# Consensys/gnark

Measured on AMD Instinct MI355X. Metric: G1 MSM throughput, BN254, 2^24 scalar-muls on one GPU (Groth16 proofs/s at 2^24 constraints in 'groth16'), higher is better.
Workload: dtype u64 Montgomery limbs in memory; 29/28-bit limbs, v_mad_u64_u32 (32x32+64) in registers

## Files before the change

### gnark_amd/csrc/msm_reduce.hip.h

```cpp
#pragma once
#include <vector>

#include "msm_lazy.hip.h"

namespace ga {

constexpr int MSM_HOT_TASKS = 16;
constexpr uint32_t MSM_VHOT_TASKS = 512;
constexpr uint32_t MSM_VHOT_SPLIT = 64;
constexpr int MSM_GROUP = 32;

template <class F>
__global__ void __launch_bounds__(64)
msm_hot_kernel(const XYZZ<F>* __restrict__ partial, const uint32_t* __restrict__ task_off,
               const uint32_t* __restrict__ hot_list, const uint32_t* __restrict__ hot_count, XYZZ<F>* __restrict__ bsum,
               uint32_t bsum_stride, uint32_t part_stride) {
    __shared__ LazyPt<F> sh[64];
    __shared__ XYZZ<F> shx[64];
    __shared__ uint32_t bad;
    partial += (uint64_t)blockIdx.y * part_stride;
    bsum += (uint64_t)blockIdx.y * bsum_stride;
    const uint32_t nh = *hot_count;
    for (uint32_t h = blockIdx.x; h < nh; h += gridDim.x) {
        const uint32_t b = hot_list[h];
        const uint32_t t0 = task_off[b], t1 = task_off[b + 1];
        block_sum29<F>(t1 - t0, [&](uint32_t i) { return &partial[t0 + i]; }, &bsum[b], sh, shx, &bad);
    }
}

template <class F>
__global__ void __launch_bounds__(64)
msm_vhot_stage1_kernel(const XYZZ<F>* __restrict__ partial, const uint32_t* __restrict__ task_off, const uint32_t* __restrict__ vhot_list,
                       const uint32_t* __restrict__ vhot_count, XYZZ<F>* __restrict__ vtmp, uint32_t part_stride, uint32_t vtmp_stride) {
    __shared__ LazyPt<F> sh[64];
    __shared__ XYZZ<F> shx[64];
    __shared__ uint32_t bad;
    partial += (uint64_t)blockIdx.y * part_stride;
    vtmp += (uint64_t)blockIdx.y * vtmp_stride;
    const uint32_t items = *vhot_count * MSM_VHOT_SPLIT;
    for (uint32_t id = blockIdx.x; id < items; id += gridDim.x) {
        const uint32_t h = id / MSM_VHOT_SPLIT, part = id % MSM_VHOT_SPLIT;
        const uint32_t b = vhot_list[h];
        const uint32_t t0 = task_off[b], t1 = task_off[b + 1];
        const uint32_t per = (t1 - t0 + MSM_VHOT_SPLIT - 1) / MSM_VHOT_SPLIT;
        const uint32_t lo = t0 + part * per < t1 ? t0 + part * per : t1;
        const uint32_t hi = lo + per < t1 ? lo + per : t1;
        block_sum29<F>(hi - lo, [&](uint32_t i) { return &partial[lo + i]; }, &vtmp[id], sh, shx, &bad);
    }
}
template <class F>
__global__ void __launch_bounds__(64)
msm_vhot_stage2_kernel(const XYZZ<F>* __restrict__ vtmp, const uint32_t* __restrict__ vhot_list, const uint32_t* __restrict__ vhot_count,
                       XYZZ<F>* __restrict__ bsum, uint32_t bsum_stride, uint32_t vtmp_stride) {
    static_assert(MSM_VHOT_SPLIT == 64, "one partial result per lane");
    __shared__ LazyPt<F> sh[64];
    __shared__ XYZZ<F> shx[64];
    __shared__ uint32_t bad;
    vtmp += (uint64_t)blockIdx.y * vtmp_stride;
    bsum += (uint64_t)blockIdx.y * bsum_stride;
    const uint32_t nv = *vhot_count;
    for (uint32_t h = blockIdx.x; h < nv; h += gridDim.x)
        block_sum29<F>(MSM_VHOT_SPLIT, [&](uint32_t i) { return &vtmp[h * MSM_VHOT_SPLIT + i]; }, &bsum[vhot_list[h]], sh, shx, &bad);
}

template <class F>
__global__ void msm_merge_kernel(const XYZZ<F>* __restrict__ partial, const uint32_t* __restrict__ task_off, uint32_t nb,
                                 XYZZ<F>* __restrict__ bsum, uint32_t* __restrict__ hot_list, uint32_t* __restrict__ hot_count,
                                 uint32_t* __restrict__ vhot_list, uint32_t* __restrict__ vhot_count, uint32_t part_stride) {
    uint32_t b = blockIdx.x * blockDim.x + threadIdx.x;
    if (b >= nb) return;
    partial += (uint64_t)blockIdx.y * part_stride;
    bsum += (uint64_t)blockIdx.y * nb;
    uint32_t t0 = task_off[b], t1 = task_off[b + 1];
    uint32_t nt = t1 - t0;
    if (nt == 1) return;
    if (nt > MSM_VHOT_TASKS) {
        if (blockIdx.y == 0) vhot_list[atomicAdd(vhot_count, 1u)] = b;
        return;
    }
    if (nt > MSM_HOT_TASKS) {
        if (blockIdx.y == 0) hot_list[atomicAdd(hot_count, 1u)] = b;
        return;
    }
    XYZZ<F> out = xyzz_inf<F>();
    bool exact = true;
    if constexpr (BaseFieldOf<F>::P::N <= 8) {
        LazyPt<F> acc;
        acc.inf = 1;
        for (uint32_t t = t0; t < t1; t++) lazy_acc<F>(acc, load_pod<XYZZ<F>>(&partial[t]));
        exact = false;
        if (!acc.inf) {
            out.zz = Lazy<F>::to_mem(acc.v.zz);
            exact = is_zero(out.zz);
            out.x = Lazy<F>::to_mem(acc.v.x);
            out.y = Lazy<F>::to_mem(acc.v.y);
            out.zzz = Lazy<F>::to_mem(acc.v.zzz);
        }
    }
    if (exact) {
        out = xyzz_inf<F>();
        for (uint32_t t = t0; t < t1; t++) out = add(out, load_pod<XYZZ<F>>(&partial[t]));
    }
    store_pod(&bsum[b], out);
}

template <class F>
__global__ void __launch_bounds__(64)
msm_reduce_groups_kernel(const XYZZ<F>* __restrict__ bsum, uint32_t half, uint32_t m, uint32_t groups_per_win,
                         uint32_t total_groups, XYZZ<F>* __restrict__ gsum) {
    uint32_t gid = blockIdx.x * blockDim.x + threadIdx.x;
    if (gid >= total_groups) return;
    uint32_t w = gid / groups_per_win, g = gid % groups_per_win;
    const XYZZ<F>* B = bsum + (uint64_t)w * half + (uint64_t)g * m;
    XYZZ<F> running = xyzz_inf<F>(), local = xyzz_inf<F>();
    for (int j = (int)m - 1; j >= 0; j--) {
        running = add(running, load_pod<XYZZ<F>>(&B[j]));
        local = add(local, running);
    }
    uint32_t base = g * m;
    if (base != 0) {
        XYZZ<F> r = xyzz_inf<F>();
        int top = 31 - __clz(base);
        for (int bit = top; bit >= 0; bit--) {
            r = dbl(r);
            if ((base >> bit) & 1) r = add(r, running);
        }
        local = add(local, r);
    }
    store_pod(&gsum[gid], local);
}

template <class F>
__global__ void __launch_bounds__(64)
msm_reduce_groups29_kernel(const XYZZ<F>* __restrict__ bsum, uint32_t half, uint32_t m, uint32_t groups_per_win,
                           uint32_t total_groups, XYZZ<F>* __restrict__ lsum, XYZZ<F>* __restrict__ rsum,
                           uint32_t* __restrict__ redo_list, uint32_t* __restrict__ redo_count) {
    uint32_t gid = blockIdx.x * blockDim.x + threadIdx.x;
    if (gid >= total_groups) return;
    uint32_t w = gid / groups_per_win, g = gid % groups_per_win;
    const XYZZ<F>* B = bsum + (uint64_t)w * half + (uint64_t)g * m;
    Lazy4<F> running, local;
    bool r_inf = true, l_inf = true;
    for (int j = (int)m - 1; j >= 0; j--) {
        XYZZ<F> b = load_pod<XYZZ<F>>(&B[j]);
        if (!is_inf(b)) {
            Lazy4<F> lb = lazy4_from_mem<F>(b);
            if (r_inf) {
                running = lb;
                r_inf = false;
            } else {
                add29<F>(running, lb);
            }
        }
        if (!r_inf) {
            if (l_inf) {
                local = running;
                l_inf = false;
            } else {
                add29<F>(local, running);
            }
        }
    }
    XYZZ<F> lo = xyzz_inf<F>(), ro = xyzz_inf<F>();
    bool bad = false;
    if (!r_inf) {
        ro.zz = Lazy<F>::to_mem(running.zz);
        lo.zz = Lazy<F>::to_mem(local.zz);
        bad = is_zero(ro.zz) | is_zero(lo.zz);
        ro.x = Lazy<F>::to_mem(running.x);
        ro.y = Lazy<F>::to_mem(running.y);
        ro.zzz = Lazy<F>::to_mem(running.zzz);
        lo.x = Lazy<F>::to_mem(local.x);
        lo.y = Lazy<F>::to_mem(local.y);
        lo.zzz = Lazy<F>::to_mem(local.zzz);
    }
    if (bad) {
        redo_list[atomicAdd(redo_count, 1u)] = gid;
        return;
    }
    store_pod(&lsum[gid], lo);
    store_pod(&rsum[gid], ro);
}

template <class F>
__global__ void __launch_bounds__(64)
msm_reduce_groups_redo_kernel(const XYZZ<F>* __restrict__ bsum, uint32_t half, uint32_t m, uint32_t groups_per_win,
                              const uint32_t* __restrict__ redo_list, const uint32_t* __restrict__ redo_count,
                              XYZZ<F>* __restrict__ lsum, XYZZ<F>* __restrict__ rsum) {
    const uint32_t nredo = *redo_count;
    for (uint32_t r = blockIdx.x * blockDim.x + threadIdx.x; r < nredo; r += gridDim.x * blockDim.x) {
        const uint32_t gid = redo_list[r];
        uint32_t w = gid / groups_per_win, g = gid % groups_per_win;
        const XYZZ<F>* B = bsum + (uint64_t)w * half + (uint64_t)g * m;
        XYZZ<F> running = xyzz_inf<F>(), local = xyzz_inf<F>();
        for (int j = (int)m - 1; j >= 0; j--) {
            running = add(running, load_pod<XYZZ<F>>(&B[j]));
            local = add(local, running);
        }
        store_pod(&lsum[gid], local);
        store_pod(&rsum[gid], running);
    }
}

template <class F>
__global__ void __launch_bounds__(64)
msm_bit_partial_kernel(const XYZZ<F>* __restrict__ rsum, const XYZZ<F>* __restrict__ lsum, uint32_t groups_per_win,
                       uint32_t chunk_len, int log_chunk, XYZZ<F>* __restrict__ part) {
    __shared__ LazyPt<F> sh[64];
    __shared__ XYZZ<F> shx[64];
    __shared__ uint32_t bad;
    const uint32_t ch = blockIdx.x, b = blockIdx.y, w = blockIdx.z;
    const uint32_t nbits = gridDim.y, chunks = gridDim.x;
    const uint32_t base = ch * chunk_len;
    const XYZZ<F>* R = rsum + (uint64_t)w * groups_per_win;
    XYZZ<F>* dst = &part[((uint64_t)w * nbits + b) * chunks + ch];
    if (b == nbits - 1) {
        const XYZZ<F>* Lp = lsum + (uint64_t)w * groups_per_win;
        block_sum29<F>(chunk_len, [&](uint32_t i) { return &Lp[base + i]; }, dst, sh, shx, &bad);
    } else if ((int)b >= log_chunk) {
        block_sum29<F>(((base >> b) & 1) ? chunk_len : 0u, [&](uint32_t i) { return &R[base + i]; }, dst, sh, shx, &bad);
    } else {
        block_sum29<F>(chunk_len / 2, [&](uint32_t i) { return &R[base + (((i >> b) << (b + 1)) | (1u << b) | (i & ((1u << b) - 1)))]; }, dst, sh,
                       shx, &bad);
    }
}

template <class F>
__global__ void __launch_bounds__(64)
msm_segment_sum29_kernel(const XYZZ<F>* __restrict__ in, uint32_t seg_len, XYZZ<F>* __restrict__ out) {
    __shared__ LazyPt<F> sh[64];
    __shared__ XYZZ<F> shx[64];
    __shared__ uint32_t bad;
    const uint64_t base = (uint64_t)blockIdx.x * seg_len;
    block_sum29<F>(seg_len, [&](uint32_t i) { return &in[base + i]; }, &out[blockIdx.x], sh, shx, &bad);
}

template <class F>
__global__ void __launch_bounds__(64)
msm_segment_sum_kernel(const XYZZ<F>* __restrict__ in, uint32_t seg_len, XYZZ<F>* __restrict__ out) {
    __shared__ XYZZ<F> sh[64];
    const uint64_t base = (uint64_t)blockIdx.x * seg_len;
    XYZZ<F> acc = xyzz_inf<F>();
    for (uint32_t g = threadIdx.x; g < seg_len; g += 64) acc = add(acc, load_pod<XYZZ<F>>(&in[base + g]));
    acc = wave_tree_sum(acc, sh);
    if (threadIdx.x == 0) store_pod(&out[blockIdx.x], acc);
}

struct MsmReducePlan {
    int nsets;
    uint32_t m_groups;
    uint32_t groups_per_win, total_groups;
    bool big_set, lazy;
};
inline MsmReducePlan msm_reduce_plan(Ctx* ctx, const void* d_bases, const MsmPrepared& P, int ntab) {
    MsmReducePlan R;
    const uint32_t half = P.half;
    R.nsets = ntab > 1 ? ntab : P.nsets;
    const int tuned_group = ctx->tun.msm_group.load(std::memory_order_relaxed);
    R.m_groups = tuned_group ? (uint32_t)tuned_group : (uint32_t)MSM_GROUP;
    const uint64_t min_lanes = 32768;
    while (R.m_groups > 2 && (uint64_t)half * R.nsets / R.m_groups < min_lanes) R.m_groups >>= 1;
    if (R.m_groups > half) R.m_groups = half;
    R.groups_per_win = half / R.m_groups;
    R.total_groups = R.groups_per_win * R.nsets;
    R.big_set = (uint64_t)half * R.nsets >= ctx->tun.reduce_lazy_min;
    const bool dense_set = P.m >= 16ull * (uint64_t)half * (uint64_t)P.nsets && !(P.table && ctx->is_sparse_set(d_bases));
    R.lazy = R.big_set || dense_set;
    return R;
}

template <class F>
struct MsmMerge {
    uint32_t *hot_list, *hot_count, *vhot_list;
    XYZZ<F>* vtmp;
    uint32_t vtmp_stride;
};
template <class F>
int msm_merge_scratch(Ctx* ctx, const MsmPrepared& P, int ntab, hipStream_t st, MsmMerge<F>* M) {
    const uint64_t vhot_cap = P.max_tasks / MSM_VHOT_TASKS + 2;
    GA_CHECK(ctx->scratch_get("msm_hot", ((uint64_t)P.nb + 2) * 4, (void**)&M->hot_list));
    GA_CHECK(ctx->scratch_get("msm_hot_count", 256, (void**)&M->hot_count));
    GA_CHECK(ctx->scratch_get("msm_vhot", vhot_cap * 4, (void**)&M->vhot_list));
    GA_CHECK(ctx->scratch_get("msm_vhot_tmp", (uint64_t)ntab * vhot_cap * MSM_VHOT_SPLIT * sizeof(XYZZ<F>), (void**)&M->vtmp));
    M->vtmp_stride = (uint32_t)(vhot_cap * MSM_VHOT_SPLIT);
    GA_HIP_CHECK(hipMemsetAsync(M->hot_count, 0, 8, st));
    return GA_OK;
}
template <class F>
int msm_merge(Ctx* ctx, const MsmPrepared& P, int ntab, hipStream_t st, const MsmMerge<F>& M, XYZZ<F>* sums) {
    StageTimer tm(ctx, "msm_merge");
    const uint32_t nb = P.nb, part_stride = (uint32_t)P.max_tasks;
    const unsigned ny = (unsigned)ntab;
    XYZZ<F>* bsum = sums;
    const XYZZ<F>* partial = sums + (uint64_t)ntab * nb;
    const uint32_t *task_off = P.task_off, *hot_count = M.hot_count, *vhot_count = M.hot_count + 1;
    hipLaunchKernelGGL((msm_merge_kernel<F>), dim3((nb + 255) / 256, ny), dim3(256), 0, st, partial, task_off, nb, bsum, M.hot_list, M.hot_count,
                       M.vhot_list, M.hot_count + 1, part_stride);
    hipLaunchKernelGGL((msm_hot_kernel<F>), dim3(512, ny), dim3(64), 0, st, partial, task_off, (const uint32_t*)M.hot_list, hot_count, bsum, nb,
                       part_stride);
    hipLaunchKernelGGL((msm_vhot_stage1_kernel<F>), dim3(2048, ny), dim3(64), 0, st, partial, task_off, (const uint32_t*)M.vhot_list, vhot_count,
                       M.vtmp, part_stride, M.vtmp_stride);
    hipLaunchKernelGGL((msm_vhot_stage2_kernel<F>), dim3(256, ny), dim3(64), 0, st, (const XYZZ<F>*)M.vtmp, (const uint32_t*)M.vhot_list,
                       vhot_count, bsum, nb, M.vtmp_stride);
    GA_KERNEL_CHECK();
    return GA_OK;
}

template <class F>
struct MsmRows {
    const XYZZ<F>* d = nullptr;
    int per_set = 1;
    const uint32_t* flagged_groups = nullptr;
};

template <class F>
int msm_reduce_exact(Ctx* ctx, const MsmReducePlan& R, uint32_t half, const XYZZ<F>* bsum, hipStream_t st, MsmRows<F>* rows) {
    XYZZ<F>*gsum, *gsum2, *wsum;
    GA_CHECK(ctx->scratch_get("msm_gsum", (uint64_t)R.total_groups * sizeof(XYZZ<F>), (void**)&gsum));
    GA_CHECK(ctx->scratch_get("msm_gsum2", ((uint64_t)R.total_groups / 1024 + 64) * sizeof(XYZZ<F>), (void**)&gsum2));
    GA_CHECK(ctx->scratch_get("msm_wsum", (uint64_t)R.nsets * sizeof(XYZZ<F>), (void**)&wsum));
    StageTimer tm(ctx, "msm_reduce");
    hipLaunchKernelGGL((msm_reduce_groups_kernel<F>), dim3((R.total_groups + 63) / 64), dim3(64), 0, st, bsum, half, R.m_groups, R.groups_per_win,
                       R.total_groups, gsum);
    const uint32_t sg = 1024;
    if (R.groups_per_win > 2 * sg) {
        const uint32_t nseg = R.groups_per_win / sg;
        hipLaunchKernelGGL((msm_segment_sum_kernel<F>), dim3(nseg * R.nsets), dim3(64), 0, st, (const XYZZ<F>*)gsum, sg, gsum2);
        hipLaunchKernelGGL((msm_segment_sum_kernel<F>), dim3(R.nsets), dim3(64), 0, st, (const XYZZ<F>*)gsum2, nseg, wsum);
    } else {
        hipLaunchKernelGGL((msm_segment_sum_kernel<F>), dim3(R.nsets), dim3(64), 0, st, (const XYZZ<F>*)gsum, R.groups_per_win, wsum);
    }
    GA_KERNEL_CHECK();
    rows->d = wsum;
    return GA_OK;
}

template <class F>
int msm_reduce_lazy(Ctx* ctx, const MsmReducePlan& R, uint32_t half, const XYZZ<F>* bsum, hipStream_t st, MsmRows<F>* rows) {
    const int nbits = ilog2_u64(R.groups_per_win), nsets = R.nsets;
    uint32_t sg = 1024;
    while (sg > 64 && (uint64_t)(R.groups_per_win / sg) * (uint64_t)(nbits + 1) * (uint64_t)nsets < 2048) sg >>= 1;
    const uint32_t chunk_len = R.groups_per_win > sg ? sg : R.groups_per_win;
    const uint32_t chunks = R.groups_per_win / chunk_len;
    const int log_chunk = ilog2_u64(chunk_len);
    XYZZ<F>*gsum, *rsum, *bpart, *bits;
    uint32_t *rg_list, *rg_count;
    GA_CHECK(ctx->scratch_get("msm_gsum", (uint64_t)R.total_groups * sizeof(XYZZ<F>), (void**)&gsum));
    GA_CHECK(ctx->scratch_get("msm_rsum", (uint64_t)R.total_groups * sizeof(XYZZ<F>), (void**)&rsum));
    GA_CHECK(ctx->scratch_get("msm_bpart", ((uint64_t)nsets * (nbits + 1) * chunks + 64) * sizeof(XYZZ<F>), (void**)&bpart));
    GA_CHECK(ctx->scratch_get("msm_bits", ((uint64_t)nsets * (nbits + 1) + 64) * sizeof(XYZZ<F>), (void**)&bits));
    GA_CHECK(ctx->scratch_get("msm_redo_groups", ((uint64_t)R.total_groups + 2) * 4, (void**)&rg_list));
    GA_CHECK(ctx->scratch_get("msm_redo_groups_count", 256, (void**)&rg_count));
    GA_HIP_CHECK(hipMemsetAsync(rg_count, 0, 4, st));
    StageTimer tm(ctx, "msm_reduce");
    hipLaunchKernelGGL((msm_reduce_groups29_kernel<F>), dim3((R.total_groups + 63) / 64), dim3(64), 0, st, bsum, half, R.m_groups,
                       R.groups_per_win, R.total_groups, gsum, rsum, rg_list, rg_count);
    hipLaunchKernelGGL((msm_reduce_groups_redo_kernel<F>), dim3(256), dim3(64), 0, st, bsum, half, R.m_groups, R.groups_per_win,
                       (const uint32_t*)rg_list, (const uint32_t*)rg_count, gsum, rsum);
    hipLaunchKernelGGL((msm_bit_partial_kernel<F>), dim3(chunks, (unsigned)nbits + 1, (unsigned)nsets), dim3(64), 0, st,
                       (const XYZZ<F>*)rsum, (const XYZZ<F>*)gsum, R.groups_per_win, chunk_len, log_chunk, bpart);
    hipLaunchKernelGGL((msm_segment_sum29_kernel<F>), dim3((unsigned)(nsets * (nbits + 1))), dim3(64), 0, st, (const XYZZ<F>*)bpart,
                       chunks, bits);
    GA_KERNEL_CHECK();
    rows->d = bits;
    rows->per_set = nbits + 1;
    rows->flagged_groups = rg_count;
    return GA_OK;
}

template <class F>
XYZZ<F> msm_combine_horner(const XYZZ<F>* ws, int nsets, int c) {
    XYZZ<F> acc = xyzz_inf<F>();
    for (int w = nsets - 1; w >= 0; w--) {
        for (int k = 0; k < c; k++) acc = dbl(acc);
        acc = add(acc, ws[w]);
    }
    return acc;
}
template <class F>
XYZZ<F> msm_combine_set(const XYZZ<F>* hb, int nbits, int log_m) {
    XYZZ<F> acc = xyzz_inf<F>();
    for (int b = nbits - 1; b >= 0; b--) acc = add(dbl(acc), hb[b]);
    for (int k = 0; k < log_m; k++) acc = dbl(acc);
    return add(hb[nbits], acc);
}
template <class F>
XYZZ<F> msm_combine_descent(const XYZZ<F>* hb, int nsets, int nbits, int log_m, int c) {
    const int rows = nbits + 1, top = c * (nsets - 1) + log_m + nbits - 1;
    std::vector<std::vector<const XYZZ<F>*>> at((size_t)top + 1);
    for (int w = 0; w < nsets; w++) {
        at[(size_t)(c * w)].push_back(&hb[(size_t)w * rows + nbits]);
        for (int b = 0; b < nbits; b++) at[(size_t)(c * w + log_m + b)].push_back(&hb[(size_t)w * rows + b]);
    }
    XYZZ<F> acc = xyzz_inf<F>();
    for (int pos = top; pos >= 0; pos--) {
        if (pos != top) acc = dbl(acc);
        for (const XYZZ<F>* t : at[(size_t)pos]) acc = add(acc, *t);
    }
    return acc;
}
template <class F>
void msm_combine(const MsmReducePlan& R, const XYZZ<F>* h, int per_set, int horner_c, XYZZ<F>* out) {
    const int nbits = per_set - 1, log_m = ilog2_u64(R.m_groups);
    if (!R.lazy) {
        if (horner_c > 0) out[0] = msm_combine_horner(h, R.nsets, horner_c);
        else
            for (int w = 0; w < R.nsets; w++) out[w] = h[w];
    } else if (horner_c > 0) {
        out[0] = msm_combine_descent(h, R.nsets, nbits, log_m, horner_c);
    } else {
        for (int w = 0; w < R.nsets; w++) out[w] = msm_combine_set(h + (size_t)w * per_set, nbits, log_m);
    }
}

}
```

Before: 912.9.

## Compact warm buckets before merging and dedupe high-bit partial sums

The merge step is split into a classify kernel and a merge kernel. The classify kernel builds a warm-bucket list using wave-ballot compaction. The merge kernel then walks only that list, so lanes no longer diverge across buckets with 1, hot, or very-hot task counts, and lazy failures are sent to the hot path instead of an exact serial re-add. The bit-partial stage no longer runs one full row per high bit, most of them empty. It computes a single full-chunk row and lets the final kernel choose chunks by bit, which cuts the partial grid from nbits+1 rows to log_chunk+2. Both changes add extra launches and atomics, and the hot list is now sized per table.

Result: no change. 918.6 (median of 6 runs) (+0.6%).

```diff
diff --git a/gnark_amd/csrc/msm_reduce.hip.h b/gnark_amd/csrc/msm_reduce.hip.h
--- a/gnark_amd/csrc/msm_reduce.hip.h
+++ b/gnark_amd/csrc/msm_reduce.hip.h
@@ -64,44 +64,53 @@
 }
 
 template <class F>
-__global__ void msm_merge_kernel(const XYZZ<F>* __restrict__ partial, const uint32_t* __restrict__ task_off, uint32_t nb,
-                                 XYZZ<F>* __restrict__ bsum, uint32_t* __restrict__ hot_list, uint32_t* __restrict__ hot_count,
-                                 uint32_t* __restrict__ vhot_list, uint32_t* __restrict__ vhot_count, uint32_t part_stride) {
-    uint32_t b = blockIdx.x * blockDim.x + threadIdx.x;
-    if (b >= nb) return;
+__global__ void __launch_bounds__(256)
+msm_merge_classify_kernel(const uint32_t* __restrict__ task_off, uint32_t nb, XYZZ<F>* __restrict__ bsum, uint32_t* __restrict__ warm_list,
+                          uint32_t* __restrict__ warm_count, uint32_t* __restrict__ hot_list, uint32_t* __restrict__ hot_count,
+                          uint32_t* __restrict__ vhot_list, uint32_t* __restrict__ vhot_count) {
+    const uint32_t b = blockIdx.x * blockDim.x + threadIdx.x;
+    const uint32_t nt = b < nb ? task_off[b + 1] - task_off[b] : 1;
+    if (nt == 0) store_pod(&bsum[(uint64_t)blockIdx.y * nb + b], xyzz_inf<F>());
+    if (blockIdx.y != 0) return;
+    if (nt > MSM_VHOT_TASKS) vhot_list[atomicAdd(vhot_count, 1u)] = b;
+    else if (nt > (uint32_t)MSM_HOT_TASKS) hot_list[atomicAdd(hot_count, 1u)] = b;
+    const bool warm = nt >= 2 && nt <= (uint32_t)MSM_HOT_TASKS;
+    const unsigned long long mask = __ballot(warm);
+    if (mask == 0) return;
+    const int lane = threadIdx.x & 63, leader = __ffsll(mask) - 1;
+    uint32_t base = 0;
+    if (lane == leader) base = atomicAdd(warm_count, (uint32_t)__popcll(mask));
+    base = __shfl(base, leader);
+    if (warm) warm_list[base + (uint32_t)__popcll(mask & ((1ull << lane) - 1))] = b;
+}
+
+template <class F>
+__global__ void __launch_bounds__(64)
+msm_merge_warm_kernel(const XYZZ<F>* __restrict__ partial, const uint32_t* __restrict__ task_off, const uint32_t* __restrict__ warm_list,
+                      const uint32_t* __restrict__ warm_count, XYZZ<F>* __restrict__ bsum, uint32_t bsum_stride, uint32_t part_stride,
+                      uint32_t* __restrict__ hot_list, uint32_t* __restrict__ hot_count) {
     partial += (uint64_t)blockIdx.y * part_stride;
-    bsum += (uint64_t)blockIdx.y * nb;
-    uint32_t t0 = task_off[b], t1 = task_off[b + 1];
-    uint32_t nt = t1 - t0;
-    if (nt == 1) return;
-    if (nt > MSM_VHOT_TASKS) {
-        if (blockIdx.y == 0) vhot_list[atomicAdd(vhot_count, 1u)] = b;
-        return;
-    }
-    if (nt > MSM_HOT_TASKS) {
-        if (blockIdx.y == 0) hot_list[atomicAdd(hot_count, 1u)] = b;
-        return;
-    }
-    XYZZ<F> out = xyzz_inf<F>();
-    bool exact = true;
-    if constexpr (BaseFieldOf<F>::P::N <= 8) {
+    bsum += (uint64_t)blockIdx.y * bsum_stride;
+    const uint32_t nw = *warm_count;
+    for (uint32_t h = blockIdx.x * blockDim.x + threadIdx.x; h < nw; h += gridDim.x * blockDim.x) {
+        const uint32_t b = warm_list[h];
+        const uint32_t t0 = task_off[b], t1 = task_off[b + 1];
         LazyPt<F> acc;
         acc.inf = 1;
         for (uint32_t t = t0; t < t1; t++) lazy_acc<F>(acc, load_pod<XYZZ<F>>(&partial[t]));
-        exact = false;
+        XYZZ<F> out = xyzz_inf<F>();
         if (!acc.inf) {
             out.zz = Lazy<F>::to_mem(acc.v.zz);
-            exact = is_zero(out.zz);
+            if (is_zero(out.zz)) {
+                hot_list[atomicAdd(hot_count, 1u)] = b;
+                continue;
+            }
             out.x = Lazy<F>::to_mem(acc.v.x);
             out.y = Lazy<F>::to_mem(acc.v.y);
             out.zzz = Lazy<F>::to_mem(acc.v.zzz);
         }
-    }
-    if (exact) {
-        out = xyzz_inf<F>();
-        for (uint32_t t = t0; t < t1; t++) out = add(out, load_pod<XYZZ<F>>(&partial[t]));
-    }
-    store_pod(&bsum[b], out);
+        store_pod(&bsum[b], out);
+    }
 }
 
 template <class F>
@@ -202,6 +211,8 @@
     }
 }
 
+__device__ __forceinline__ uint32_t insert_one_bit(uint32_t i, uint32_t b) { return ((i >> b) << (b + 1)) | (1u << b) | (i & ((1u << b) - 1)); }
+
 template <class F>
 __global__ void __launch_bounds__(64)
 msm_bit_partial_kernel(const XYZZ<F>* __restrict__ rsum, const XYZZ<F>* __restrict__ lsum, uint32_t groups_per_win,
@@ -209,30 +220,41 @@
     __shared__ LazyPt<F> sh[64];
     __shared__ XYZZ<F> shx[64];
     __shared__ uint32_t bad;
-    const uint32_t ch = blockIdx.x, b = blockIdx.y, w = blockIdx.z;
-    const uint32_t nbits = gridDim.y, chunks = gridDim.x;
+    const uint32_t ch = blockIdx.x, r = blockIdx.y, w = blockIdx.z;
+    const uint32_t rows = gridDim.y, chunks = gridDim.x;
     const uint32_t base = ch * chunk_len;
     const XYZZ<F>* R = rsum + (uint64_t)w * groups_per_win;
-    XYZZ<F>* dst = &part[((uint64_t)w * nbits + b) * chunks + ch];
-    if (b == nbits - 1) {
+    XYZZ<F>* dst = &part[((uint64_t)w * rows + r) * chunks + ch];
+    if ((int)r == log_chunk + 1) {
         const XYZZ<F>* Lp = lsum + (uint64_t)w * groups_per_win;
         block_sum29<F>(chunk_len, [&](uint32_t i) { return &Lp[base + i]; }, dst, sh, shx, &bad);
-    } else if ((int)b >= log_chunk) {
-        block_sum29<F>(((base >> b) & 1) ? chunk_len : 0u, [&](uint32_t i) { return &R[base + i]; }, dst, sh, shx, &bad);
+    } else if ((int)r == log_chunk) {
+        block_sum29<F>(chunk_len, [&](uint32_t i) { return &R[base + i]; }, dst, sh, shx, &bad);
     } else {
-        block_sum29<F>(chunk_len / 2, [&](uint32_t i) { return &R[base + (((i >> b) << (b + 1)) | (1u << b) | (i & ((1u << b) - 1)))]; }, dst, sh,
-                       shx, &bad);
-    }
-}
-
-template <class F>
-__global__ void __launch_bounds__(64)
-msm_segment_sum29_kernel(const XYZZ<F>* __restrict__ in, uint32_t seg_len, XYZZ<F>* __restrict__ out) {
+        block_sum29<F>(chunk_len / 2, [&](uint32_t i) { return &R[base + insert_one_bit(i, r)]; }, dst, sh, shx, &bad);
+    }
+}
+
+template <class F>
+__global__ void __launch_bounds__(64)
+msm_bit_final_kernel(const XYZZ<F>* __restrict__ part, uint32_t chunks, int log_chunk, XYZZ<F>* __restrict__ bits) {
     __shared__ LazyPt<F> sh[64];
     __shared__ XYZZ<F> shx[64];
     __shared__ uint32_t bad;
-    const uint64_t base = (uint64_t)blockIdx.x * seg_len;
-    block_sum29<F>(seg_len, [&](uint32_t i) { return &in[base + i]; }, &out[blockIdx.x], sh, shx, &bad);
+    const uint32_t b = blockIdx.x, w = blockIdx.y, nbits = gridDim.x - 1;
+    const XYZZ<F>* P = part + (uint64_t)w * (log_chunk + 2) * chunks;
+    XYZZ<F>* dst = &bits[(uint64_t)w * (nbits + 1) + b];
+    if (b == nbits) {
+        const XYZZ<F>* row = P + (uint64_t)(log_chunk + 1) * chunks;
+        block_sum29<F>(chunks, [&](uint32_t i) { return &row[i]; }, dst, sh, shx, &bad);
+    } else if ((int)b < log_chunk) {
+        const XYZZ<F>* row = P + (uint64_t)b * chunks;
+        block_sum29<F>(chunks, [&](uint32_t i) { return &row[i]; }, dst, sh, shx, &bad);
+    } else {
+        const XYZZ<F>* row = P + (uint64_t)log_chunk * chunks;
+        const uint32_t cb = b - (uint32_t)log_chunk;
+        block_sum29<F>(chunks / 2, [&](uint32_t i) { return &row[insert_one_bit(i, cb)]; }, dst, sh, shx, &bad);
+    }
 }
 
 template <class F>
@@ -271,19 +293,20 @@
 
 template <class F>
 struct MsmMerge {
-    uint32_t *hot_list, *hot_count, *vhot_list;
+    uint32_t *hot_list, *hot_count, *vhot_list, *warm_list;
     XYZZ<F>* vtmp;
     uint32_t vtmp_stride;
 };
 template <class F>
 int msm_merge_scratch(Ctx* ctx, const MsmPrepared& P, int ntab, hipStream_t st, MsmMerge<F>* M) {
     const uint64_t vhot_cap = P.max_tasks / MSM_VHOT_TASKS + 2;
-    GA_CHECK(ctx->scratch_get("msm_hot", ((uint64_t)P.nb + 2) * 4, (void**)&M->hot_list));
+    GA_CHECK(ctx->scratch_get("msm_hot", ((uint64_t)P.nb * ntab + 2) * 4, (void**)&M->hot_list));
+    GA_CHECK(ctx->scratch_get("msm_warm", ((uint64_t)P.nb + 2) * 4, (void**)&M->warm_list));
     GA_CHECK(ctx->scratch_get("msm_hot_count", 256, (void**)&M->hot_count));
     GA_CHECK(ctx->scratch_get("msm_vhot", vhot_cap * 4, (void**)&M->vhot_list));
     GA_CHECK(ctx->scratch_get("msm_vhot_tmp", (uint64_t)ntab * vhot_cap * MSM_VHOT_SPLIT * sizeof(XYZZ<F>), (void**)&M->vtmp));
     M->vtmp_stride = (uint32_t)(vhot_cap * MSM_VHOT_SPLIT);
-    GA_HIP_CHECK(hipMemsetAsync(M->hot_count, 0, 8, st));
+    GA_HIP_CHECK(hipMemsetAsync(M->hot_count, 0, 12, st));
     return GA_OK;
 }
 template <class F>
@@ -293,9 +316,11 @@
     const unsigned ny = (unsigned)ntab;
     XYZZ<F>* bsum = sums;
     const XYZZ<F>* partial = sums + (uint64_t)ntab * nb;
-    const uint32_t *task_off = P.task_off, *hot_count = M.hot_count, *vhot_count = M.hot_count + 1;
-    hipLaunchKernelGGL((msm_merge_kernel<F>), dim3((nb + 255) / 256, ny), dim3(256), 0, st, partial, task_off, nb, bsum, M.hot_list, M.hot_count,
-                       M.vhot_list, M.hot_count + 1, part_stride);
+    const uint32_t *task_off = P.task_off, *hot_count = M.hot_count, *vhot_count = M.hot_count + 1, *warm_count = M.hot_count + 2;
+    hipLaunchKernelGGL((msm_merge_classify_kernel<F>), dim3((nb + 255) / 256, ny), dim3(256), 0, st, task_off, nb, bsum, M.warm_list, M.hot_count + 2,
+                       M.hot_list, M.hot_count, M.vhot_list, M.hot_count + 1);
+    hipLaunchKernelGGL((msm_merge_warm_kernel<F>), dim3(4096, ny), dim3(64), 0, st, partial, task_off, (const uint32_t*)M.warm_list, warm_count, bsum,
+                       nb, part_stride, M.hot_list, M.hot_count);
     hipLaunchKernelGGL((msm_hot_kernel<F>), dim3(512, ny), dim3(64), 0, st, partial, task_off, (const uint32_t*)M.hot_list, hot_count, bsum, nb,
                        part_stride);
     hipLaunchKernelGGL((msm_vhot_stage1_kernel<F>), dim3(2048, ny), dim3(64), 0, st, partial, task_off, (const uint32_t*)M.vhot_list, vhot_count,
@@ -347,7 +372,7 @@
     uint32_t *rg_list, *rg_count;
     GA_CHECK(ctx->scratch_get("msm_gsum", (uint64_t)R.total_groups * sizeof(XYZZ<F>), (void**)&gsum));
     GA_CHECK(ctx->scratch_get("msm_rsum", (uint64_t)R.total_groups * sizeof(XYZZ<F>), (void**)&rsum));
-    GA_CHECK(ctx->scratch_get("msm_bpart", ((uint64_t)nsets * (nbits + 1) * chunks + 64) * sizeof(XYZZ<F>), (void**)&bpart));
+    GA_CHECK(ctx->scratch_get("msm_bpart", ((uint64_t)nsets * (log_chunk + 2) * chunks + 64) * sizeof(XYZZ<F>), (void**)&bpart));
     GA_CHECK(ctx->scratch_get("msm_bits", ((uint64_t)nsets * (nbits + 1) + 64) * sizeof(XYZZ<F>), (void**)&bits));
     GA_CHECK(ctx->scratch_get("msm_redo_groups", ((uint64_t)R.total_groups + 2) * 4, (void**)&rg_list));
     GA_CHECK(ctx->scratch_get("msm_redo_groups_count", 256, (void**)&rg_count));
@@ -357,10 +382,10 @@
                        R.groups_per_win, R.total_groups, gsum, rsum, rg_list, rg_count);
     hipLaunchKernelGGL((msm_reduce_groups_redo_kernel<F>), dim3(256), dim3(64), 0, st, bsum, half, R.m_groups, R.groups_per_win,
                        (const uint32_t*)rg_list, (const uint32_t*)rg_count, gsum, rsum);
-    hipLaunchKernelGGL((msm_bit_partial_kernel<F>), dim3(chunks, (unsigned)nbits + 1, (unsigned)nsets), dim3(64), 0, st,
+    hipLaunchKernelGGL((msm_bit_partial_kernel<F>), dim3(chunks, (unsigned)log_chunk + 2, (unsigned)nsets), dim3(64), 0, st,
                        (const XYZZ<F>*)rsum, (const XYZZ<F>*)gsum, R.groups_per_win, chunk_len, log_chunk, bpart);
-    hipLaunchKernelGGL((msm_segment_sum29_kernel<F>), dim3((unsigned)(nsets * (nbits + 1))), dim3(64), 0, st, (const XYZZ<F>*)bpart,
-                       chunks, bits);
+    hipLaunchKernelGGL((msm_bit_final_kernel<F>), dim3((unsigned)nbits + 1, (unsigned)nsets), dim3(64), 0, st, (const XYZZ<F>*)bpart, chunks,
+                       log_chunk, bits);
     GA_KERNEL_CHECK();
     rows->d = bits;
     rows->per_set = nbits + 1;
```
